# geobacter-rs/rav1e

Hardware: AMD Instinct MI355X
Metric: encoded frames/sec + Mpixels/sec, 4K 8-bit speed=10, 1/2/4/8 GPU vs host CPU (higher is better)
Workload: dtype u8

## Files before the change

### rav1e_amd/csrc/rv_chain.h

```cpp
#pragma once

#include "rv_device.h"

namespace rv {

__host__ __device__ inline rv_mv qfull(rv_mv m) {
  return rv_mv{(int16_t)((m.row / 8) * 8), (int16_t)((m.col / 8) * 8)};
}

__host__ __device__ inline rv_mc_job mc_job_for(const rv_plane &p, int po_x, int po_y, rv_mv mv,
                                       int dst_x, int dst_y) {
  const int ys = 3 + p.ydec, xs = 3 + p.xdec;
  const int roff = (int)mv.row >> ys, coff = (int)mv.col >> xs;
  rv_mc_job m;
  m.row_frac = ((int)mv.row - (roff << ys)) << (4 - ys);
  m.col_frac = ((int)mv.col - (coff << xs)) << (4 - xs);
  m.src_x = clampi(po_x + coff - 3, -p.xorigin, p.width) + 3;
  m.src_y = clampi(po_y + roff - 3, -p.yorigin, p.height) + 3;
  m.dst_x = dst_x;
  m.dst_y = dst_y;
  return m;
}

enum ChainMode {
// ... 4 lines not shown
struct ChainNext {
  int mode;
  rv_ds_job *jobs;
};

__device__ inline void chain_emit(const ChainNext &c, int job, int n_per_ref, int n_refs,
                                  rv_mv best) {
  (void)n_per_ref;
  (void)n_refs;
  if (c.mode == kChainFullToSub) c.jobs[job].pred[0] = best;
}

struct MvStack {
  int32_t n[2];
  rv_mv s[2][2];
  rv_mv c[2][2];
};

struct CandGeo {
  int nsb, tw, th, tx0, ty0, tws, ths;
  int R;
  int M;
  int comp;
  const MvStack *stk;
};

enum CandMode { kNearestMv = 0, kNear0Mv = 1, kGlobalMv = 2, kNewMv = 3, kCandModes = 4 };
enum CompMode {
  kGlobalGlobal = 0, kNearestNearest = 1, kNewNew = 2, kNearestNew = 3, kNewNearest = 4,
  kNearNear = 5, kCompModes = 6
};

__host__ __device__ inline bool mv_eq(rv_mv a, rv_mv b) { return a.row == b.row && a.col == b.col; }

__host__ __device__ inline int cand_stack(const CandGeo &g, const rv_fs_result *sub, int sb,
                                          int k, rv_mv &s0, rv_mv &s1) {
  if (g.stk) {
    const MvStack &m = g.stk[sb];
    s0 = m.s[k][0];
    s1 = m.s[k][1];
    return m.n[k];
  }
  const int sx = sb % g.tw, sy = sb / g.tw;
  const int fx = g.tx0 + sx, fy = g.ty0 + sy;
  const bool up = sy > 0 && fy % g.ths != 0, left = sx > 0 && fx % g.tws != 0;
  const rv_mv zero{0, 0};
  const rv_mv a = up ? sub[k * g.nsb + sb - g.tw].best_mv : zero;
  const rv_mv l = left ? sub[k * g.nsb + sb - 1].best_mv : zero;
  if (up) {
    s0 = a;
    s1 = l;
    return left && !mv_eq(l, a) ? 2 : 1;
  }
  s0 = l;
  s1 = zero;
  return left ? 1 : 0;
}

__host__ __device__ inline int comp_stack(const CandGeo &g, const rv_fs_result *sub, int sb,
                                          rv_mv &e00, rv_mv &e01, rv_mv &e10, rv_mv &e11) {
  if (g.stk) {
    const MvStack &m = g.stk[sb];
    e00 = m.c[0][0];
    e01 = m.c[0][1];
    e10 = m.c[1][0];
    e11 = m.c[1][1];
    return 2;
  }
  const int sx = sb % g.tw, sy = sb / g.tw;
  const int fx = g.tx0 + sx, fy = g.ty0 + sy;
  const bool up = sy > 0 && fy % g.ths != 0, left = sx > 0 && fx % g.tws != 0;
  const rv_mv zero{0, 0};
  const rv_mv a0 = up ? sub[sb - g.tw].best_mv : zero, a1 = up ? sub[g.nsb + sb - g.tw].best_mv : zero;
  const rv_mv l0 = left ? sub[sb - 1].best_mv : zero, l1 = left ? sub[g.nsb + sb - 1].best_mv : zero;
  e10 = e11 = zero;
  if (up) {
    e00 = a0;
    e01 = a1;
    if (left && (!mv_eq(l0, a0) || !mv_eq(l1, a1))) {
      e10 = l0;
      e11 = l1;
      return 2;
    }
    return 1;
  }
  e00 = l0;
  e01 = l1;
  return left ? 1 : 0;
}

__host__ __device__ inline void comp_mvs(const CandGeo &g, const rv_fs_result *sub, int sb, int m,
                                         rv_mv *mv0, rv_mv *mv1) {
  rv_mv e00, e01, e10, e11;
  const int n = comp_stack(g, sub, sb, e00, e01, e10, e11);
  const rv_mv zero{0, 0};
  const rv_mv me0 = sub[sb].best_mv, me1 = sub[g.nsb + sb].best_mv;
  const rv_mv n00 = n >= 1 ? e00 : zero, n01 = n >= 1 ? e01 : zero;
  switch (m) {
    case kGlobalGlobal:
      *mv0 = *mv1 = zero;
      break;
    case kNearestNearest:
      *mv0 = n00;
      *mv1 = n01;
      break;
    case kNewNew:
      *mv0 = me0;
      *mv1 = me1;
      break;
    case kNearestNew:
      *mv0 = n00;
      *mv1 = me1;
      break;
    case kNewNearest:
      *mv0 = me0;
      *mv1 = n01;
      break;
    default:
      *mv0 = n >= 2 ? e10 : zero;
      *mv1 = n >= 2 ? e11 : zero;
      break;
  }
}

__host__ __device__ inline bool cand_mv(const CandGeo &g, const rv_fs_result *sub, int sb, int c,
                                        rv_mv *mv) {
  const int k = c / g.M, m = c - k * g.M;
  rv_mv s0, s1;
  const int n = cand_stack(g, sub, sb, k, s0, s1);
  const rv_mv zero{0, 0};
  switch (m) {
    case kNearestMv:
      *mv = n >= 1 ? s0 : zero;
      return true;
    case kNear0Mv:
      *mv = n >= 2 ? s1 : zero;
      return n >= 1;
    case kGlobalMv:
      *mv = zero;
      return n >= 2;
    default: {
      const rv_mv me = sub[k * g.nsb + sb].best_mv;
      *mv = me;
      return !(n >= 1 && mv_eq(s0, me)) && !(n >= 2 && mv_eq(s1, me)) &&
             (me.row != 0 || me.col != 0);
    }
  }
}

__host__ __device__ inline bool cand_live(const CandGeo &g, const rv_fs_result *sub, int sb, int c,
                                          rv_mv *mv) {
  if (!cand_mv(g, sub, sb, c, mv)) return false;
  for (int c2 = (c / g.M) * g.M; c2 < c; c2++) {
    rv_mv m2;
    if (cand_mv(g, sub, sb, c2, &m2) && mv_eq(m2, *mv)) return false;
  }
  return true;
}
__host__ __device__ inline bool comp_live(const CandGeo &g, const rv_fs_result *sub, int sb, int m) {
  rv_mv a0, a1;
  comp_mvs(g, sub, sb, m, &a0, &a1);
  for (int m2 = 0; m2 < m; m2++) {
// ... 9 lines not shown
```

### rav1e_amd/csrc/rv_rdo.h

```cpp
#pragma once

#include "rv_chain.h"
#include "rv_device.h"
#include "rv_quant.h"

namespace rv {

struct RdoPlane {
  rv_plane org;
  rv_plane ref[2];
  rv_plane dst;
  int32_t *levels;
  uint64_t *out;
  QCtx q;
};

struct RdoWinner {
  int32_t c;
  int32_t skip;
  double cost;
  uint64_t dist;
};

struct RdoArgs {
// ... 6 lines not shown
  int n_tx;
  int cand_base;
  const int32_t *list;
  const int32_t *count;
  int commit;
  int ntx_per_cand;
  int bd;
  int bsize;
  int mb_w, mb_h;
  int sub_w, sub_h;
  int xdec, ydec;
  int q_tx_index;
  int tx_size, qindex;
  const void *iedges;
  const uint8_t *imodes;
  const uint8_t *iwin;
};

}

int rv_quant_ctx(int qindex, int tx_area, int is_intra, int bit_depth, int dc_delta_q,
                 int ac_delta_q, rv::QCtx *out);

int rv_rdo_candidates(const rv::RdoArgs &luma, const rv::RdoArgs &chroma, int hbd,
                      hipStream_t s, bool compound = false);

int rv_rdo_blocks2(const rv::RdoArgs &l, const rv::RdoArgs &c, int nl, int nc, int hbd,
                   hipStream_t s, int mode);
int rv_rdo_blocks(const rv::RdoArgs &a, bool luma, int nplanes, int n_tx_size, int hbd,
                  hipStream_t s, int mode);

int rv_rdo_args_put(const rv::RdoArgs *h, int n, rv::RdoArgs *dev, hipStream_t s);
int rv_rdo_candidates_list(const rv::RdoArgs *h, const rv::RdoArgs *dev, int nsets, int mode_a,
                           int hbd, hipStream_t s, int max_grid = 0, uint32_t *kp_cnt = nullptr,
                           unsigned long long *kp_t = nullptr);

int rv_rdo_intra(const rv::RdoArgs &luma, const rv::RdoArgs &chroma, int hbd, hipStream_t s);
```

### rav1e_amd/csrc/rv_rdo.hip

```cpp
#include <stdio.h>
#include <stdlib.h>
#include <string.h>

#include <type_traits>

#include "rv_distortion.h"
#include "rv_intra.h"
#include "rv_rdo.h"
#include "rv_tx.h"

namespace rv {


__constant__ int8_t kRdoReg[2][16][8] = {
    {{0, 0, 0, 127, 0, 0, 0, 0}, {0, 2, -6, 126, 8, -2, 0, 0},
     {0, 2, -10, 122, 18, -4, 0, 0}, {0, 2, -12, 116, 28, -8, 2, 0},
     {0, 2, -14, 110, 38, -10, 2, 0}, {0, 2, -14, 102, 48, -12, 2, 0},
     {0, 2, -16, 94, 58, -12, 2, 0}, {0, 2, -14, 84, 66, -12, 2, 0},
     {0, 2, -14, 76, 76, -14, 2, 0}, {0, 2, -12, 66, 84, -14, 2, 0},
     {0, 2, -12, 58, 94, -16, 2, 0}, {0, 2, -12, 48, 102, -14, 2, 0},
     {0, 2, -10, 38, 110, -14, 2, 0}, {0, 2, -8, 28, 116, -12, 2, 0},
     {0, 0, -4, 18, 122, -10, 2, 0}, {0, 0, -2, 8, 126, -6, 2, 0}},
    {{0, 0, 0, 127, 0, 0, 0, 0}, {0, 0, -4, 126, 8, -2, 0, 0},
     {0, 0, -8, 122, 18, -4, 0, 0}, {0, 0, -10, 116, 28, -6, 0, 0},
// ... 64 lines not shown
  const int tsx = fx % a.g.tws, tsy = fy % a.g.ths;
  j.ivar = tsx == 0 && tsy == 0 ? 0 : tsy == 0 ? 1 : tsx == 0 ? 2 : 3;
  j.imode = mode;
  j.iedge = (const uint8_t *)a.iedges + ((size_t)sb * 3 + plane) * kIntraEdge * sizeof(Px);
  j.bx = (fx * a.bsize) >> a.xdec;
  j.by = (fy * a.bsize) >> a.ydec;
  j.ox = j.oy = 0;
  j.src_x = j.src_y = j.cf = j.rf = j.ref = 0;
  j.src2_x = j.src2_y = j.cf2 = j.rf2 = 0;
  j.comp = false;
  j.zero = false;
  return j;
}

template <typename Px, int N, int G>
__device__ __forceinline__ void intra_fill(const RdoJob &jb, int32_t *e, Px *pred, int bd, int lane) {
  const Px *eg = (const Px *)jb.iedge;
  for (int i = lane; i < kIntraEdge; i += G) e[i] = eg[i];
  wave_sync();
  IntraSetup st = intra_setup(jb.imode, jb.ivar);
  if (st.mode == 0) st.dcv = intra_dc<G>(e, jb.ivar, N, N, bd, lane);
  const int maxv = (1 << bd) - 1;
  for (int i = lane; i < N * N; i += G) {
    const int r = i / N, c = i - r * N;
    pred[i] = (Px)intra_px(st, e, N, N, r, c, maxv);
  }
  wave_sync();
}

__device__ __forceinline__ int rdo_ntx(const RdoArgs &a) {
  return a.count ? __builtin_amdgcn_readfirstlane(*a.count) * a.ntx_per_cand : a.n_tx;
}

template <int N>
__device__ __forceinline__ RdoJob rdo_job(const RdoArgs &a, const RdoPlane &pl, int t) {
  const int ci = t / a.ntx_per_cand, sub = t - ci * a.ntx_per_cand;
  const int cand = a.list ? a.list[ci] : a.cand_base + ci;
  int sb, c;
  RdoJob j;
  j.zero = false;
  j.oi = cand * a.ntx_per_cand + sub;
  if (a.commit) {
    sb = cand;
    c = a.win[sb].c;
    j.zero = a.win[sb].skip != 0;
  } else {
    c = cand / a.g.nsb;
    sb = cand - c * a.g.nsb;
  }
  rv_mv mv, mv1{0, 0};
  j.comp = c >= a.g.R * a.g.M;
  if (j.comp) {
    comp_mvs(a.g, a.sub, sb, c - a.g.R * a.g.M, &mv, &mv1);
    j.ref = 0;
  } else {
    (void)cand_mv(a.g, a.sub, sb, c, &mv);
    j.ref = c / a.g.M;
  }
  const int sx = sb % a.g.tw, sy = sb / a.g.tw;
  j.bx = ((a.g.tx0 + sx) * a.bsize) >> a.xdec;
  j.by = ((a.g.ty0 + sy) * a.bsize) >> a.ydec;
  const int txc = a.mb_w / N;
  j.ox = (sub % txc) * N;
  j.oy = (sub / txc) * N;
  const rv_mc_job m = mc_job_for(pl.ref[j.ref], j.bx, j.by, mv, 0, 0);
  j.src_x = m.src_x;
  j.src_y = m.src_y;
  j.cf = m.col_frac;
  j.rf = m.row_frac;
  j.src2_x = j.src2_y = j.cf2 = j.rf2 = 0;
  if (j.comp) {
    const rv_mc_job m1 = mc_job_for(pl.ref[1], j.bx, j.by, mv1, 0, 0);
    j.src2_x = m1.src_x;
    j.src2_y = m1.src_y;
    j.cf2 = m1.col_frac;
    j.rf2 = m1.row_frac;
  }
  return j;
}

struct McF {
  uint32_t xp[3];
  int xsum;
  int yt[8];
  int cf, rf;
};
template <typename Px>
__device__ __forceinline__ McF mc_setup(int cf, int rf, int w, int h) {
  McF f;
// ... 181 lines not shown
        ss2 += (uint32_t)wmul24(sv, sv);
        sd2 += (uint32_t)wmul24(e, e);
        ssd += (uint32_t)wmul24(sv, e);
      }
#pragma unroll
      for (int m = 1; m < 8; m <<= 1) {
        ss += __shfl_xor(ss, m, 64);
        sd += __shfl_xor(sd, m, 64);
        ss2 += __shfl_xor(ss2, m, 64);
        sd2 += __shfl_xor(sd2, m, 64);
        ssd += __shfl_xor(ssd, m, 64);
      }
      if (row == 0) {
        const uint64_t v = cdef_dist_finish(ss, sd, ss2, sd2, ssd, a.bd);
        const int px = j.bx + j.ox + bx * 8, py = j.by + j.oy + by * 8;
        acc += distortion_biased(v, rdo_bias(a, px >> 2, py >> 2));
      }
    }
    return acc;
  } else {
    return rdo_sse_biased<Px, N, LPB>(a, j, o, os, d);
  }
}

template <typename Px, int N>
__host__ __device__ constexpr int rdo_slab_bytes() {
  constexpr int B = (int)sizeof(Px);
  constexpr int P = B == 1 ? ((N + 8 + 15) / 16) * 16 : ((2 * (N + 8) + 15) / 16) * 16;
  constexpr int RB = N < 16 ? N : 16;
  constexpr int a = N * (N + 1) * 4, b = (N + 7) * P, c = 2 * (RB + 7) * P;
  return ((a > b ? a : b) > c ? (a > b ? a : b) : c);
}

template <typename Px, int N, int LPB, int MODE, bool LUMA = false>
__device__ __forceinline__ void rdo_cand_body(const RdoArgs &a, const RdoPlane &pl, int t,
                                              bool valid, int32_t *buf, Px *pred,
                                              const uint16_t *scan) {
  constexpr int B = (int)sizeof(Px);
  constexpr int S = N + 1;
  constexpr int G = LPB / N, RG = N / G;
  constexpr int U = RG < 8 ? RG : 8;
  constexpr int P = B == 1 ? ((N + 8 + 15) / 16) * 16 : ((2 * (N + 8) + 15) / 16) * 16;
  constexpr int C32 = N < 32 ? N : 32;
  static_assert(!LUMA || N >= 8, "cdef distortion runs on 8x8 blocks");
  const int lane = rv_tid() & (LPB - 1);
  RdoJob jb;
  if constexpr (MODE == 3)
    jb = rdo_job_intra<Px, N>(a, &pl == &a.p[1] ? 2 : 1, t);
  else
    jb = rdo_job<N>(a, pl, t);
  const rv_plane &ref = pl.ref[jb.ref];
  const int ox = jb.ox, oy = jb.oy;
  const int bd = a.bd, ib = bd == 12 ? 2 : 4, maxv = (1 << bd) - 1;
  const int sx0 = jb.bx + ox, sy0 = jb.by + oy;
  auto wave_sync = [] {
    __builtin_amdgcn_fence(__ATOMIC_RELEASE, "wavefront");
    __builtin_amdgcn_wave_barrier();
    __builtin_amdgcn_fence(__ATOMIC_ACQUIRE, "wavefront");
  };

  if constexpr (MODE == 3) {
    intra_fill<Px, N, LPB>(jb, buf, pred, a.bd, lane);
  } else if (MODE == 1 || (MODE == 2 && jb.comp)) {
    static_assert(2 * (16 + 7) * (sizeof(Px) == 1 ? 48 : 80) <= N * (N + 1) * 4 || N != 32,
                  "compound windows must fit the coefficient slab");
    mc_compound<Px, N, (N < 16 ? N : 16)>(a, pl, jb, reinterpret_cast<uint32_t *>(buf), pred);
  } else
  {
    uint32_t *win = reinterpret_cast<uint32_t *>(buf);
    const uint8_t *sp = (const uint8_t *)plane_ptr<Px>(ref, jb.src_x + ox - 3, jb.src_y + oy - 3);
    const int64_t rs = (int64_t)ref.stride * B;
    constexpr int kRowDw = ((N + 7) * B + 3) / 4;
    constexpr int kTot = (N + 7) * kRowDw;
#pragma unroll 4
    for (int i = lane; i < kTot; i += LPB) {
      const int r = i / kRowDw, d = i - r * kRowDw;
      uint32_t v;
      __builtin_memcpy(&v, sp + r * rs + 4 * d, 4);
      win[r * (P / 4) + d] = B == 1 ? v ^ 0x80808080u : v;
    }
    wave_sync();
    const int cf = jb.cf, rf = jb.rf;
    const int8_t *xf = kRdoReg[a.mb_w <= 4][cf];
// ... 454 lines not shown
  }
  const uint64_t d = luma_dist<Px>(a, jb, plane_ptr<Px>(pl.org, jb.bx, jb.by), pl.org.stride, pred);
  if (valid && lane == 0) pl.out[(int64_t)jb.oi * 3 + 1] = d;
}

template <typename Px, typename Mid, int NPART, int MODE>
__device__ __forceinline__ void rdo_luma_body(const RdoArgs &a, const RdoPlane &pl, int t,
                                              uint8_t *scr, Px *pred, const uint16_t *scan) {
  const int lane = rv_tid() & 63;
  RdoJob jb;
  if constexpr (MODE == 3)
    jb = rdo_job_intra<Px, 64>(a, 0, t);
  else
    jb = rdo_job<64>(a, pl, t);
  luma_front<Px, NPART, MODE>(a, pl, t, jb, true, scr, pred);
  wave_sync();
  int32_t *fmid = reinterpret_cast<int32_t *>(scr);
  if (lane < 16) luma_fwd_row(fmid + lane * 65, a.bd);
  wave_sync();
  luma_quantize(a, pl, t, jb, true, fmid, scan);
  wave_sync();
  const int range = a.bd + 8, crange = a.bd + 6 > 16 ? a.bd + 6 : 16;
  Mid *imid = reinterpret_cast<Mid *>(scr);
  {
    int32_t v[64];
    if (lane < 32) luma_inv_row_load(fmid, lane, v, range, nullptr);
    wave_sync();
    if (lane < 32) luma_inv_row_tx(v, imid + lane * 66, range, crange);
  }
  wave_sync();
  luma_back<Px, Mid>(a, pl, t, jb, true, imid, pred);
}

template <typename Px, int MODE>
__device__ __forceinline__ void rdo_chroma_pair(const RdoArgs &chroma, int b, int32_t *buf,
                                                Px *pred, const uint16_t *scan, int pairs = -1) {
  if (pairs < 0) pairs = (chroma.n_tx + 1) / 2;
  const int plane = b / pairs;
  const int half = (rv_tid() & 63) >> 5;
  const int n = rdo_ntx(chroma);
  int i = 2 * (b - plane * pairs) + half;
  if (i - half >= n) return;
  const bool valid = i < n;
  if (!valid) i -= 1;
  rdo_cand_body<Px, 32, 32, MODE>(chroma, chroma.p[plane], i, valid, buf + half * 32 * 33,
                            pred + half * 32 * 32, scan);
}

__device__ __forceinline__ void stage_scan(uint16_t *dst, int tx_index) {
  const uint16_t *src = RV_SCANS + RV_SCAN_OFF[tx_index];
  for (int i = rv_tid(); i < 1024; i += blockDim.x) dst[i] = src[i];
  __syncthreads();
}

template <typename Px>
using SingleLds = LumaLds<Px, typename std::conditional<sizeof(Px) == 1, int16_t, int32_t>::type, 2>;
constexpr int kChromaPair(int pxb) { return 2 * 32 * 33 * 4 + 2 * 32 * 32 * pxb; }

template <typename Px, int MODE>
__global__ __launch_bounds__(64) __attribute__((amdgpu_waves_per_eu(4))) void rdo_frame_kernel(
    RdoArgs luma, RdoArgs chroma) {
  using L = SingleLds<Px>;
  using Mid = typename std::conditional<sizeof(Px) == 1, int16_t, int32_t>::type;
  __shared__ __align__(16) uint8_t lds[cmax(L::kSlot, kChromaPair(sizeof(Px)))];
  __shared__ uint16_t scan[1024];
  const int b = blockIdx.x;
  stage_scan(scan, b < luma.n_tx ? luma.q_tx_index : chroma.q_tx_index);
  if (b < luma.n_tx && b >= rdo_ntx(luma)) return;
  if (b < luma.n_tx)
    rdo_luma_body<Px, Mid, 2, MODE>(luma, luma.p[0], b, lds,
                              reinterpret_cast<Px *>(lds + L::kScr), scan);
  else
    rdo_chroma_pair<Px, MODE>(chroma, b - luma.n_tx, reinterpret_cast<int32_t *>(lds),
                        reinterpret_cast<Px *>(lds + 2 * 32 * 33 * 4), scan);
}

template <typename Px>
struct QuadLds {
  using L = LumaLds<Px, int16_t, sizeof(Px) == 1 ? 2 : 4>;
  static constexpr int kBytes = cmax(4 * L::kSlot, 3 * kChromaPair(sizeof(Px)));
};

#ifndef RV_RDO_PHASES
#define RV_RDO_PHASES 0
#endif
__device__ unsigned long long g_rdo_ph[3][8];
struct QuadPh {
  unsigned long long t[5];
};

template <typename Px, int MODE>
__device__ __forceinline__ void rdo_quad_luma(const RdoArgs &luma, int b, int n, int var,
                                              uint8_t *lds, const uint16_t *scan,
                                              QuadPh *ph = nullptr) {
  using L = typename QuadLds<Px>::L;
  constexpr int NPART = sizeof(Px) == 1 ? 2 : 4;
  const int wave = __builtin_amdgcn_readfirstlane(rv_tid() >> 6), lane = rv_tid() & 63;
  auto slot = [&](int q) __attribute__((always_inline)) { return lds + q * L::kSlot; };
  auto fmid = [&](int q) __attribute__((always_inline)) {
    return reinterpret_cast<int32_t *>(slot(q));
  };
  auto imid = [&](int q) __attribute__((always_inline)) {
    return reinterpret_cast<int16_t *>(slot(q));
  };
  auto pred = [&](int q) __attribute__((always_inline)) {
    return reinterpret_cast<Px *>(slot(q) + L::kScr);
  };
  const int t0 = 4 * b, t = t0 + wave;
  if (t0 >= n) return;
  const bool valid = t < n;
  RdoJob jb;
  if constexpr (MODE == 3)
    jb = rdo_job_intra<Px, 64>(luma, 0, valid ? t : n - 1);
  else
    jb = rdo_job<64>(luma, luma.p[0], valid ? t : n - 1);
  const bool late_dist = (var & 1) && !luma.commit;
  const bool prio = (var & 2) != 0;
  if (valid)
    luma_front<Px, NPART, MODE>(luma, luma.p[0], t, jb, true, slot(wave), pred(wave), !late_dist);
  __syncthreads();
  if (RV_RDO_PHASES && ph) ph->t[1] = wall_clock64();
  if (wave == 0) {
    if (prio) __builtin_amdgcn_s_setprio(2);
    const int q = lane >> 4;
    if (t0 + q < n) luma_fwd_row(fmid(q) + (lane & 15) * 65, luma.bd);
    if (prio) __builtin_amdgcn_s_setprio(0);
  } else if (late_dist && valid) {
    const uint64_t d = luma_dist<Px>(luma, jb, plane_ptr<Px>(luma.p[0].org, jb.bx, jb.by),
                                     luma.p[0].org.stride, pred(wave));
    if (lane == 0) luma.p[0].out[(int64_t)jb.oi * 3 + 0] = d;
  }
  __syncthreads();
  if (RV_RDO_PHASES && ph) ph->t[2] = wall_clock64();
  if (valid) luma_quantize(luma, luma.p[0], t, jb, true, fmid(wave), scan);
  __syncthreads();
  if (RV_RDO_PHASES && ph) ph->t[3] = wall_clock64();
  if (wave < 2) {
    if (prio) __builtin_amdgcn_s_setprio(2);
    const int q = 2 * wave + (lane >> 5), rr = lane & 31;
    const bool vq = t0 + q < n;
    const int range = luma.bd + 8, crange = luma.bd + 6 > 16 ? luma.bd + 6 : 16;
    int32_t v[64];
    if (vq) luma_inv_row_load(fmid(q), rr, v, range, nullptr);
    wave_sync();
    if (vq) luma_inv_row_tx(v, imid(q) + rr * 66, range, crange);
    if (prio) __builtin_amdgcn_s_setprio(0);
  } else if (wave == 2 && late_dist) {
    RdoJob j0;
    if constexpr (MODE == 3)
      j0 = rdo_job_intra<Px, 64>(luma, 0, t0);
    else
      j0 = rdo_job<64>(luma, luma.p[0], t0);
    const uint64_t d = luma_dist<Px>(luma, j0, plane_ptr<Px>(luma.p[0].org, j0.bx, j0.by),
                                     luma.p[0].org.stride, pred(0));
    if (lane == 0) luma.p[0].out[(int64_t)j0.oi * 3 + 0] = d;
  }
  __syncthreads();
  if (RV_RDO_PHASES && ph) ph->t[4] = wall_clock64();
  if (valid) luma_back<Px, int16_t>(luma, luma.p[0], t, jb, true, imid(wave), pred(wave));
}

template <typename Px, int MODE>
__device__ __forceinline__ void rdo_quad_chroma(const RdoArgs &chroma, int c, int pairs,
                                                uint8_t *lds, const uint16_t *scan) {
  const int wave = __builtin_amdgcn_readfirstlane(rv_tid() >> 6);
  const int pair = 3 * c + wave;
  if (wave == 3 || pair >= 2 * pairs) return;
  uint8_t *w = lds + wave * kChromaPair(sizeof(Px));
  rdo_chroma_pair<Px, MODE>(chroma, pair, reinterpret_cast<int32_t *>(w),
                            reinterpret_cast<Px *>(w + 2 * 32 * 33 * 4), scan, pairs);
}

template <typename Px, int MODE>
__device__ __forceinline__ void rdo_quad_chroma4(const RdoArgs &chroma, int c, int n, uint8_t *lds,
                                                 const uint16_t *scan) {
  constexpr int kSlab = rdo_slab_bytes<Px, 32>();
  static_assert(4 * (kSlab + 32 * 32 * (int)sizeof(Px)) <= QuadLds<Px>::kBytes, "4 chroma slabs");
  const int wave = __builtin_amdgcn_readfirstlane(rv_tid() >> 6);
  const int k = 4 * c + wave;
  if (k >= 2 * n) return;
  const int plane = k >= n ? 1 : 0, i = k - plane * n;
  uint8_t *w = lds + wave * (kSlab + 32 * 32 * (int)sizeof(Px));
  rdo_cand_body<Px, 32, 64, MODE>(chroma, chroma.p[plane], i, true, reinterpret_cast<int32_t *>(w),
                                  reinterpret_cast<Px *>(w + kSlab), scan);
}

template <typename Px, int MODE>
__device__ __forceinline__ void rdo_quad_wg(RdoArgs luma, RdoArgs chroma, int nquads,
                                            int var, int b, uint8_t *lds, uint16_t *scan) {
  if (b >= nquads) {
    const int pairs = (chroma.n_tx + 1) / 2, nc = rdo_ntx(chroma);
    bool any = false;
    for (int w = 0; w < 3; w++) {
      const int p = 3 * (b - nquads) + w;
      if (p < 2 * pairs) any |= 2 * (p - (p / pairs) * pairs) < nc;
    }
    if (!any) return;
  } else if (4 * b >= rdo_ntx(luma)) {
    return;
  }
  stage_scan(scan, b >= nquads ? chroma.q_tx_index : luma.q_tx_index);
  if (b >= nquads)
    rdo_quad_chroma<Px, MODE>(chroma, b - nquads, (chroma.n_tx + 1) / 2, lds, scan);
  else
    rdo_quad_luma<Px, MODE>(luma, b, rdo_ntx(luma), var, lds, scan);
}

template <typename Px, int MODE>
__global__ __launch_bounds__(256) __attribute__((amdgpu_waves_per_eu(4))) void rdo_quad_kernel(
    RdoArgs luma, RdoArgs chroma, int nquads, int var) {
  __shared__ __align__(16) uint8_t lds[QuadLds<Px>::kBytes];
  __shared__ uint16_t scan[1024];
  rdo_quad_wg<Px, MODE>(luma, chroma, nquads, var, blockIdx.x, lds, scan);
}

template <typename Px, int MA, int MB>
__global__ __launch_bounds__(256) __attribute__((amdgpu_waves_per_eu(4))) void rdo_quad_list_kernel(
    const RdoArgs *__restrict__ A, int nsets, int var, uint32_t *kp_cnt, unsigned long long *kp_t) {
  __shared__ __align__(16) uint8_t lds[QuadLds<Px>::kBytes];
  __shared__ uint16_t scan[1024];
  if (kp_t && threadIdx.x == 0) atomicMin(kp_t, (unsigned long long)wall_clock64());
  const RdoArgs &la = A[0], &ca = A[1], &lb = A[2], &cb = A[3];
  const int na = rdo_ntx(la), ma = rdo_ntx(ca);
  const int nb = nsets > 1 ? rdo_ntx(lb) : 0, mb = nsets > 1 ? rdo_ntx(cb) : 0;
  if (kp_cnt && blockIdx.x == 0 && threadIdx.x == 0) {
    atomicAdd(kp_cnt + (MA ? 1 : 0), (uint32_t)na);
    atomicAdd(kp_cnt + (MA ? 3 : 2), (uint32_t)ma);
    if (nsets > 1) {
      atomicAdd(kp_cnt + (MB ? 1 : 0), (uint32_t)nb);
      atomicAdd(kp_cnt + (MB ? 3 : 2), (uint32_t)mb);
    }
  }
  const int pa = (ma + 1) / 2, pb = (mb + 1) / 2;
  const bool c4 = (var & 32) != 0;
  const int e0 = (na + 3) / 4, e1 = e0 + (c4 ? (2 * ma + 3) / 4 : (2 * pa + 2) / 3);
  const int e2 = e1 + (nb + 3) / 4, e3 = e2 + (c4 ? (2 * mb + 3) / 4 : (2 * pb + 2) / 3);
  const bool phd = RV_RDO_PHASES && (var & 16) && rv_tid() == 0;
  for (int b = blockIdx.x; b < e3; b += gridDim.x) {
    QuadPh ph;
    ph.t[0] = phd ? wall_clock64() : 0;
    QuadPh *pp = phd ? &ph : nullptr;
    int set = 2;
    if (b < e0) {
      stage_scan(scan, la.q_tx_index);
      rdo_quad_luma<Px, MA>(la, b, na, var, lds, scan, pp);
      set = MA;
    } else if (b < e1) {
      stage_scan(scan, ca.q_tx_index);
      if (c4)
        rdo_quad_chroma4<Px, MA>(ca, b - e0, ma, lds, scan);
      else
        rdo_quad_chroma<Px, MA>(ca, b - e0, pa, lds, scan);
    } else if (b < e2) {
      stage_scan(scan, lb.q_tx_index);
      rdo_quad_luma<Px, MB>(lb, b - e1, nb, var, lds, scan, pp);
      set = MB;
    } else {
      stage_scan(scan, cb.q_tx_index);
      if (c4)
        rdo_quad_chroma4<Px, MB>(cb, b - e2, mb, lds, scan);
      else
        rdo_quad_chroma<Px, MB>(cb, b - e2, pb, lds, scan);
    }
    __syncthreads();
    if (phd) {
      const unsigned long long te = wall_clock64();
      if (set < 2) {
        for (int k = 0; k < 4; k++) atomicAdd(&g_rdo_ph[set][k], ph.t[k + 1] - ph.t[k]);
        atomicAdd(&g_rdo_ph[set][4], te - ph.t[4]);
      } else {
        atomicAdd(&g_rdo_ph[2][0], te - ph.t[0]);
      }
      atomicAdd(&g_rdo_ph[set][5], 1ull);
    }
  }
  if (kp_t && threadIdx.x == 0) atomicMax(kp_t + 1, (unsigned long long)wall_clock64());
}

__global__ __launch_bounds__(256) void rdo_args_store_kernel(RdoArgs a0, RdoArgs a1, RdoArgs a2,
                                                              RdoArgs a3, int n, RdoArgs *out) {
  static_assert(sizeof(RdoArgs) % 4 == 0, "word copy");
  constexpr int W = (int)(sizeof(RdoArgs) / 4);
  for (int i = threadIdx.x; i < n * W; i += blockDim.x) {
    const int k = i / W, w = i - k * W;
    const RdoArgs *s = k == 0 ? &a0 : k == 1 ? &a1 : k == 2 ? &a2 : &a3;
    uint32_t v;
    __builtin_memcpy(&v, reinterpret_cast<const uint8_t *>(s) + 4 * w, 4);
    __builtin_memcpy(reinterpret_cast<uint8_t *>(out + k) + 4 * w, &v, 4);
  }
}

constexpr unsigned kF4Pool = 1024;
constexpr int kRdoVariant = 3;

}

using namespace rv;

template <typename Px, int N, int MODE, bool LUMA>
__global__ __launch_bounds__(256) void rdo_small_kernel(RdoArgs a, int nplanes) {
  constexpr int TPW = 64 / N;
  constexpr int SLAB = rdo_slab_bytes<Px, N>();
  constexpr int PER = (SLAB + N * N * (int)sizeof(Px) + 15) / 16 * 16;
  __shared__ __align__(16) uint8_t lds[4 * TPW * PER];
  __shared__ uint16_t scan[1024];
  stage_scan(scan, a.q_tx_index);
  const int wave = rv_tid() >> 6, g = (rv_tid() & 63) / N;
  const int n = rdo_ntx(a), total = n * nplanes;
  const int w0 = (blockIdx.x * 4 + wave) * TPW;
  if (w0 >= total) return;
  const int i = w0 + g;
  const bool valid = i < total;
  const int ii = valid ? i : total - 1;
  const int plane = ii / n, t = ii - plane * n;
  uint8_t *mine = lds + (wave * TPW + g) * PER;
  rdo_cand_body<Px, N, N, MODE, LUMA>(a, a.p[plane], t, valid, reinterpret_cast<int32_t *>(mine),
                                       reinterpret_cast<Px *>(mine + SLAB), scan);
}

template <typename Px, int N, int MODE, bool LUMA>
__device__ __forceinline__ void rdo_small_part(const RdoArgs &a, int nplanes, int blk,
                                               uint8_t *lds, uint16_t *scan) {
  constexpr int TPW = 64 / N;
  constexpr int SLAB = rdo_slab_bytes<Px, N>();
  constexpr int PER = (SLAB + N * N * (int)sizeof(Px) + 15) / 16 * 16;
// ... 70 lines not shown
    return;
  }
  const int nquads = (luma.n_tx + 3) / 4;
  const unsigned grid = (unsigned)nquads + (cpairs + 2) / 3;
  if (grid == 0) return;
  if (hbd)
    rdo_quad_kernel<uint16_t, MODE><<<grid, 256, 0, s>>>(luma, chroma, nquads, kRdoVariant);
  else
    rdo_quad_kernel<uint8_t, MODE><<<grid, 256, 0, s>>>(luma, chroma, nquads, kRdoVariant);
}

int rv_rdo_candidates(const RdoArgs &luma, const RdoArgs &chroma, int hbd, hipStream_t s,
                      bool compound) {
  const unsigned cpairs = (unsigned)(2 * ((chroma.n_tx + 1) / 2));
  if (luma.commit)
    rdo_launch<2>(luma, chroma, hbd, s, cpairs);
  else if (compound)
    rdo_launch<1>(luma, chroma, hbd, s, cpairs);
  else
    rdo_launch<0>(luma, chroma, hbd, s, cpairs);
  RV_HIP_CHECK_LAUNCH();
  return RV_OK;
}

int rv_rdo_args_put(const RdoArgs *h, int n, RdoArgs *dev, hipStream_t s) {
  if (!h || !dev || n < 1 || n > 4) return rv_set_error(RV_EINVAL, "rv_rdo_args_put: bad arguments");
  rdo_args_store_kernel<<<1, 256, 0, s>>>(h[0], h[n > 1 ? 1 : 0], h[n > 2 ? 2 : 0], h[n > 3 ? 3 : 0],
                                          n, dev);
  RV_HIP_CHECK_LAUNCH();
  return RV_OK;
}

int rv_rdo_candidates_list(const RdoArgs *h, const RdoArgs *dev, int nsets, int mode_a, int hbd,
                           hipStream_t s, int max_grid, uint32_t *kp_cnt, unsigned long long *kp_t) {
  if (!h || !dev || nsets < 1 || nsets > 2 || mode_a < 0 || mode_a > 1 || (nsets == 2 && mode_a) ||
      h[0].commit || h[0].bd == 12)
    return rv_set_error(RV_EINVAL, "rv_rdo_candidates_list: bad arguments");
  for (int k = 0; k < 2 * nsets; k++)
    if (!h[k].list || !h[k].count)
      return rv_set_error(RV_EINVAL, "rv_rdo_candidates_list: the sets must be list-driven");
  static const bool phases = getenv("RAV1E_HIP_RDO_PHASES") && getenv("RAV1E_HIP_RDO_PHASES")[0] == '1';
  const int var = kRdoVariant | (phases && max_grid > 0 ? 16 : 0) | (max_grid > 0 ? 32 : 0);
  unsigned full = 0;
  for (int k = 0; k < nsets; k++)
    full += (unsigned)((h[2 * k].n_tx + 3) / 4) +
            ((var & 32) ? (unsigned)(2 * h[2 * k + 1].n_tx + 3) / 4
                        : (unsigned)(2 * ((h[2 * k + 1].n_tx + 1) / 2) + 2) / 3);
  unsigned grid = std::min(full, kF4Pool);
  if (max_grid > 0) grid = std::min(grid, (unsigned)max_grid);
  if (grid == 0) return RV_OK;
#define RV_LIST(PX, MA, MB) \
  rdo_quad_list_kernel<PX, MA, MB><<<grid, 256, 0, s>>>(dev, nsets, var, kp_cnt, kp_t)
  if (hbd) {
    if (nsets == 2) RV_LIST(uint16_t, 0, 1); else if (mode_a) RV_LIST(uint16_t, 1, 1); else RV_LIST(uint16_t, 0, 0);
  } else {
    if (nsets == 2) RV_LIST(uint8_t, 0, 1); else if (mode_a) RV_LIST(uint8_t, 1, 1); else RV_LIST(uint8_t, 0, 0);
  }
#undef RV_LIST
  RV_HIP_CHECK_LAUNCH();
  return RV_OK;
}

int rv_rdo_intra(const RdoArgs &luma, const RdoArgs &chroma, int hbd, hipStream_t s) {
  const unsigned cpairs = (unsigned)(2 * ((chroma.n_tx + 1) / 2));
  rdo_launch<3>(luma, chroma, hbd, s, cpairs);
  RV_HIP_CHECK_LAUNCH();
  return RV_OK;
}

int rv_rdo_blocks2(const RdoArgs &l, const RdoArgs &c, int nl, int nc, int hbd, hipStream_t s,
                   int mode) {
  if (nl == 32 && nc == 16) rdo_small2_launch<32, 16>(l, c, hbd, s, mode);
  else if (nl == 16 && nc == 8) rdo_small2_launch<16, 8>(l, c, hbd, s, mode);
  else if (nl == 8 && nc == 4) rdo_small2_launch<8, 4>(l, c, hbd, s, mode);
  else if (nl == 32 && nc == 32) rdo_small2_launch<32, 32>(l, c, hbd, s, mode);
  else if (nl == 16 && nc == 16) rdo_small2_launch<16, 16>(l, c, hbd, s, mode);
  else if (nl == 8 && nc == 8) rdo_small2_launch<8, 8>(l, c, hbd, s, mode);
  else return rv_set_error(RV_EINVAL, "rv_rdo_blocks2: sizes");
  RV_HIP_CHECK_LAUNCH();
  return RV_OK;
}

int rv_rdo_blocks(const RdoArgs &a, bool luma, int nplanes, int n_tx_size, int hbd,
                  hipStream_t s, int mode) {
  if (luma) {
    if (n_tx_size == 32) rdo_small_launch<32, true>(a, nplanes, hbd, s, mode);
    else if (n_tx_size == 16) rdo_small_launch<16, true>(a, nplanes, hbd, s, mode);
    else if (n_tx_size == 8) rdo_small_launch<8, true>(a, nplanes, hbd, s, mode);
    else return rv_set_error(RV_EINVAL, "rv_rdo_blocks: luma size");
// ... 32 lines not shown
```

### rav1e_amd/csrc/rv_replay_frame.hip

```cpp
#include "rv_replay.h"

namespace rv {

struct CandCost {
  double rs, rn;
  uint64_t ds, dn;
  int live;
};
__device__ inline CandCost cand_cost(const CandGeo &cg, double lambda, double ds_u, double ds_v,
                                     const rv_fs_result *sub, const uint64_t *lout,
                                     const uint64_t *uout, const uint64_t *vout, int ntx_c, int sb,
                                     int c) {
  CandCost k{0.0, 0.0, 0, 0, 0};
  const int ns = cg.R * cg.M;
  rv_mv mv;
  if (c < ns ? !cand_live(cg, sub, sb, c, &mv) : !comp_live(cg, sub, sb, c - ns)) return k;
  k.live = 1;
  const int64_t o = (int64_t)c * cg.nsb + sb;
  uint64_t su = 0, sv = 0, nu = 0, nv = 0;
  uint32_t rate = (uint32_t)lout[o * 3 + 2];
  for (int j = 0; j < ntx_c; j++) {
    const int64_t t = (o * ntx_c + j) * 3;
    su += uout[t];
    sv += vout[t];
// ... 972 lines not shown
      return rv_diamond_search_multi(&cur.hres, refs_h, g.R, r->jobs_half[lv], nr * 4, 16, 16, 0, 0,
                                     0, g.bd, r->half, nullptr, nullptr, st);
    RV_H(hipMemcpyAsync(r->half, r->half_l, (size_t)nr * g.R * 4 * sizeof(rv_fs_result),
                        hipMemcpyDeviceToDevice, st));
    fill_preds_kernel<<<(nr * g.R + 255) / 256, 256, 0, st>>>(r->jobs_full[lv], r->src_full,
                                                              nr * g.R, r->coarse, r->half, 0);
    return RV_OK;
  }

  int round0() {
    const bool with_lv = place == LvPlace::kRound0;
    if (f4_list) RV_R(rv_rdo_args_put(f4h, cg.comp ? 4 : 2, r->f4_args, st));
    RV_R(rv_diamond_search_multi(&cur.y, refs_y, g.R, r->jobs_full[lv], nr, 64, 64, 0, 0, 0, g.bd,
                                 r->full, ev_full, &to_sub, st, act));
    RV_R(ev(kEvF3Full));
    RV_R(kp.open(st));
    RV_R(rv_diamond_search_multi(&cur.y, refs_y, g.R, r->jobs_sub[lv], nr, 64, 64, 1,
                                 r->s6 ? 1 : 0, 0, g.bd, r->sub, ev_sub, nullptr, st, act, nullptr,
                                 nullptr, 1, nullptr, 0, kp.acc(0), kp.ts()));
    RV_R(kp.close(st));
    if (with_lv) RV_R(lv_me(st));
    const CandKeys keys0{r->cand_key, (uint32_t)(r->coded + 1), 0};
    cand_list_kernel<<<(nsingle + 255) / 256, 256, 0, st>>>(cg, r->sub, nsingle, r->cand_list,
                                                            r->cand_count, act, keys0);
    if (with_lv) lv_lists(st, false);
    if (cg.comp) {
      comp_list_kernel<<<(g.nsb * cg.comp + 255) / 256, 256, 0, st>>>(
          cg, r->sub, nsingle, r->cand_list + nsingle, r->cand_count + 1, act, keys0);
      if (with_lv) lv_lists(st, true);
    }
    RV_R(ev(kEvF3Sub));
    if (f4_list) {
      RV_R(kp.open(st, 1));
      RV_R(rv_rdo_candidates_list(f4h, r->f4_args, 1, 0, g.hbd, st, 0, kp.acc(1), kp.ts(1)));
      RV_R(kp.close(st, 1));
    } else
      RV_R(rv_rdo_candidates(f4h[0], f4h[1], g.hbd, st));
    if (with_lv) RV_R(lv_rdo(st));
    RV_R(ev(kEvF4Single));
    if (cg.comp) {
      if (f4_list) {
        RV_R(kp.open(st, 1));
        RV_R(rv_rdo_candidates_list(f4h + 2, r->f4_args + 2, 1, 1, g.hbd, st, 0, kp.acc(1), kp.ts(1)));
        RV_R(kp.close(st, 1));
      } else
        RV_R(rv_rdo_candidates(f4h[2], f4h[3], g.hbd, st, true));
      if (with_lv) RV_R(lv_rdo_comp(st));
    }
    RV_R(ev(kEvF4Comp));
    score_wave_kernel<<<(g.nsb + 3) / 4, 256, 0, st>>>(
        g, cg, L.lambda, L.ds[1], L.ds[2], r->sub, r->l_out, r->c_out, r->c_out + nct * 3, ntx_c,
        r->win, r->coarse, r->half, r->full, r->look, r->half_l, r->words, r->cand_count,
        r->tail + 2, r->cand_evals + 2 * slot * kLevels, r->leaf_count, nullptr, nullptr,
        r->exact ? r->dec_lv[lv] : nullptr, 0);
    return RV_OK;
  }

  int round_of(uint32_t q) {
    const int32_t *acnt = slot_cnt(q);
    int lg = q == q_first ? nr * g.R : 0;
    const int hint = q == q_first ? -1 : r->rr.last_count;
    const int hsb = hint >= 0 ? std::max(2 * hint, 16) : 0;
    int f4_grid = 0;
    if (hsb) {
      lg = std::min(hsb * g.R, 512);
      f4_grid = std::min(6 * hsb, 1024);
    }
    RV_R(kp.open(st));
    RV_R(rv_diamond_f2_f3(&cur.hres, refs_h, r->jobs_half[lv], r->half, ma.f2dirty, &cur.y,
                          refs_y, r->jobs_full[lv], r->full, ma.f3dirty, &to_sub, g.R, nr, g.bd,
                          mvl(q), acnt, lg, st, r->jobs_sub[lv], r->sub, kp.acc(0), kp.ts()));
    RV_R(kp.close(st));
    const int rg = hsb ? std::min(kRoundGrid, std::max((14 * hsb + 255) / 256, (hsb + 3) / 4))
                       : kRoundGrid;
    round_lists_kernel<<<rg, 256, 0, st>>>(
        cg, r->sub, nsingle, r->cand_list, r->cand_count, mvl(q), acnt,
        CandKeys{r->cand_key, (uint32_t)(r->coded + 1), 1});
    if (f4_list) {
      RV_R(kp.open(st, 1));
      RV_R(rv_rdo_candidates_list(f4h, r->f4_args, cg.comp ? 2 : 1, 0, g.hbd, st, f4_grid,
                                  kp.acc(1), kp.ts(1)));
      RV_R(kp.close(st, 1));
    } else {
      RV_R(rv_rdo_candidates(f4h[0], f4h[1], g.hbd, st));
      if (cg.comp) RV_R(rv_rdo_candidates(f4h[2], f4h[3], g.hbd, st, true));
    }
    score_wave_kernel<<<rg, 256, 0, st>>>(
        g, cg, L.lambda, L.ds[1], L.ds[2], r->sub, r->l_out, r->c_out, r->c_out + nct * 3, ntx_c,
        r->win, r->coarse, r->half, r->full, r->look, r->half_l, r->words, r->cand_count, nullptr,
        nullptr, nullptr, mvl(q), acnt, r->dec_lv[lv], 1);
    return RV_OK;
  }

  int mv_rounds_run(const uint8_t *iwas, bool *changed) {
    mv_runs++;
    q_first = r->rr.seq;
    ma.init = 0;
    ma.iwas = iwas;
    return run_rounds(
        r->rr, st, budget, [this](uint32_t q) { return check(q); },
        [this](uint32_t q) { return round_of(q); }, &r->mv_round_sum, &r->mv_reeval, changed,
        "mvref", ncoded, lv);
  }
  int rounds() {
    RV_R(join_edge_scores());
    ma.hq = r->half;
    ma.edge_ok = 1;
    tr.r0 = HostTrace::now();
    RV_R(mv_rounds_run(nullptr, nullptr));
    tr.mv = HostTrace::now();
    return RV_OK;
  }

  PartArgs part_args() const {
// ... 258 lines not shown
```

Baseline: 179.0.

## Add latency-mode F4 list kernel with lower wave occupancy and branchless MV stacks

Adds a latency variant of the RDO candidate list kernel, used for 8-bit non-first motion rounds. It compiles with amdgpu_waves_per_eu(2) instead of 4 and caps the grid at 768 workgroups instead of 1024. That variant also builds the neighbour MV stacks branchlessly through a templated BV path, which computes both candidates and selects between them rather than branching. The aim is to give each wave more registers and cut divergence and latency in the small later rounds, at the cost of fewer concurrent waves.

```diff
diff --git a/rav1e_amd/csrc/rv_chain.h b/rav1e_amd/csrc/rv_chain.h
--- a/rav1e_amd/csrc/rv_chain.h
+++ b/rav1e_amd/csrc/rv_chain.h
@@ -60,7 +60,13 @@
 };
 
 __host__ __device__ inline bool mv_eq(rv_mv a, rv_mv b) { return a.row == b.row && a.col == b.col; }
-
+__host__ __device__ inline rv_mv mv_if(bool c, const rv_mv &m) {
+  rv_mv r{0, 0};
+  if (c) r = m;
+  return r;
+}
+
+template <bool BV = false>
 __host__ __device__ inline int cand_stack(const CandGeo &g, const rv_fs_result *sub, int sb,
                                           int k, rv_mv &s0, rv_mv &s1) {
   if (g.stk) {
@@ -73,6 +79,13 @@
   const int fx = g.tx0 + sx, fy = g.ty0 + sy;
   const bool up = sy > 0 && fy % g.ths != 0, left = sx > 0 && fx % g.tws != 0;
   const rv_mv zero{0, 0};
+  if constexpr (BV) {
+    const rv_mv a = mv_if(up, sub[k * g.nsb + sb - g.tw].best_mv);
+    const rv_mv l = mv_if(left, sub[k * g.nsb + sb - 1].best_mv);
+    s0 = up ? a : l;
+    s1 = up ? l : zero;
+    return up ? (left && !mv_eq(l, a) ? 2 : 1) : left ? 1 : 0;
+  }
   const rv_mv a = up ? sub[k * g.nsb + sb - g.tw].best_mv : zero;
   const rv_mv l = left ? sub[k * g.nsb + sb - 1].best_mv : zero;
   if (up) {
@@ -85,6 +98,7 @@
   return left ? 1 : 0;
 }
 
+template <bool BV = false>
 __host__ __device__ inline int comp_stack(const CandGeo &g, const rv_fs_result *sub, int sb,
                                           rv_mv &e00, rv_mv &e01, rv_mv &e10, rv_mv &e11) {
   if (g.stk) {
@@ -99,8 +113,14 @@
   const int fx = g.tx0 + sx, fy = g.ty0 + sy;
   const bool up = sy > 0 && fy % g.ths != 0, left = sx > 0 && fx % g.tws != 0;
   const rv_mv zero{0, 0};
-  const rv_mv a0 = up ? sub[sb - g.tw].best_mv : zero, a1 = up ? sub[g.nsb + sb - g.tw].best_mv : zero;
-  const rv_mv l0 = left ? sub[sb - 1].best_mv : zero, l1 = left ? sub[g.nsb + sb - 1].best_mv : zero;
+  rv_mv a0, a1, l0, l1;
+  if constexpr (BV) {
+    a0 = mv_if(up, sub[sb - g.tw].best_mv), a1 = mv_if(up, sub[g.nsb + sb - g.tw].best_mv);
+    l0 = mv_if(left, sub[sb - 1].best_mv), l1 = mv_if(left, sub[g.nsb + sb - 1].best_mv);
+  } else {
+    a0 = up ? sub[sb - g.tw].best_mv : zero, a1 = up ? sub[g.nsb + sb - g.tw].best_mv : zero;
+    l0 = left ? sub[sb - 1].best_mv : zero, l1 = left ? sub[g.nsb + sb - 1].best_mv : zero;
+  }
   e10 = e11 = zero;
   if (up) {
     e00 = a0;
@@ -117,10 +137,11 @@
   return left ? 1 : 0;
 }
 
+template <bool BV = false>
 __host__ __device__ inline void comp_mvs(const CandGeo &g, const rv_fs_result *sub, int sb, int m,
                                          rv_mv *mv0, rv_mv *mv1) {
   rv_mv e00, e01, e10, e11;
-  const int n = comp_stack(g, sub, sb, e00, e01, e10, e11);
+  const int n = comp_stack<BV>(g, sub, sb, e00, e01, e10, e11);
   const rv_mv zero{0, 0};
   const rv_mv me0 = sub[sb].best_mv, me1 = sub[g.nsb + sb].best_mv;
   const rv_mv n00 = n >= 1 ? e00 : zero, n01 = n >= 1 ? e01 : zero;
@@ -151,11 +172,12 @@
   }
 }
 
+template <bool BV = false>
 __host__ __device__ inline bool cand_mv(const CandGeo &g, const rv_fs_result *sub, int sb, int c,
                                         rv_mv *mv) {
   const int k = c / g.M, m = c - k * g.M;
   rv_mv s0, s1;
-  const int n = cand_stack(g, sub, sb, k, s0, s1);
+  const int n = cand_stack<BV>(g, sub, sb, k, s0, s1);
   const rv_mv zero{0, 0};
   switch (m) {
     case kNearestMv:
diff --git a/rav1e_amd/csrc/rv_rdo.h b/rav1e_amd/csrc/rv_rdo.h
--- a/rav1e_amd/csrc/rv_rdo.h
+++ b/rav1e_amd/csrc/rv_rdo.h
@@ -62,7 +62,7 @@
 
 int rv_rdo_args_put(const rv::RdoArgs *h, int n, rv::RdoArgs *dev, hipStream_t s);
 int rv_rdo_candidates_list(const rv::RdoArgs *h, const rv::RdoArgs *dev, int nsets, int mode_a,
-                           int hbd, hipStream_t s, int max_grid = 0, uint32_t *kp_cnt = nullptr,
-                           unsigned long long *kp_t = nullptr);
+                           int hbd, hipStream_t s, int max_grid = 0, bool latency = false,
+                           uint32_t *kp_cnt = nullptr, unsigned long long *kp_t = nullptr);
 
 int rv_rdo_intra(const rv::RdoArgs &luma, const rv::RdoArgs &chroma, int hbd, hipStream_t s);
diff --git a/rav1e_amd/csrc/rv_rdo.hip b/rav1e_amd/csrc/rv_rdo.hip
--- a/rav1e_amd/csrc/rv_rdo.hip
+++ b/rav1e_amd/csrc/rv_rdo.hip
@@ -120,7 +120,7 @@
   return a.count ? __builtin_amdgcn_readfirstlane(*a.count) * a.ntx_per_cand : a.n_tx;
 }
 
-template <int N>
+template <int N, bool BV = false>
 __device__ __forceinline__ RdoJob rdo_job(const RdoArgs &a, const RdoPlane &pl, int t) {
   const int ci = t / a.ntx_per_cand, sub = t - ci * a.ntx_per_cand;
   const int cand = a.list ? a.list[ci] : a.cand_base + ci;
@@ -139,10 +139,10 @@
   rv_mv mv, mv1{0, 0};
   j.comp = c >= a.g.R * a.g.M;
   if (j.comp) {
-    comp_mvs(a.g, a.sub, sb, c - a.g.R * a.g.M, &mv, &mv1);
+    comp_mvs<BV>(a.g, a.sub, sb, c - a.g.R * a.g.M, &mv, &mv1);
     j.ref = 0;
   } else {
-    (void)cand_mv(a.g, a.sub, sb, c, &mv);
+    (void)cand_mv<BV>(a.g, a.sub, sb, c, &mv);
     j.ref = c / a.g.M;
   }
   const int sx = sb % a.g.tw, sy = sb / a.g.tw;
@@ -390,7 +390,7 @@
   return ((a > b ? a : b) > c ? (a > b ? a : b) : c);
 }
 
-template <typename Px, int N, int LPB, int MODE, bool LUMA = false>
+template <typename Px, int N, int LPB, int MODE, bool LUMA = false, bool BV = false>
 __device__ __forceinline__ void rdo_cand_body(const RdoArgs &a, const RdoPlane &pl, int t,
                                               bool valid, int32_t *buf, Px *pred,
                                               const uint16_t *scan) {
@@ -406,7 +406,7 @@
   if constexpr (MODE == 3)
     jb = rdo_job_intra<Px, N>(a, &pl == &a.p[1] ? 2 : 1, t);
   else
-    jb = rdo_job<N>(a, pl, t);
+    jb = rdo_job<N, BV>(a, pl, t);
   const rv_plane &ref = pl.ref[jb.ref];
   const int ox = jb.ox, oy = jb.oy;
   const int bd = a.bd, ib = bd == 12 ? 2 : 4, maxv = (1 << bd) - 1;
@@ -927,7 +927,7 @@
   luma_back<Px, Mid>(a, pl, t, jb, true, imid, pred);
 }
 
-template <typename Px, int MODE>
+template <typename Px, int MODE, bool BV = false>
 __device__ __forceinline__ void rdo_chroma_pair(const RdoArgs &chroma, int b, int32_t *buf,
                                                 Px *pred, const uint16_t *scan, int pairs = -1) {
   if (pairs < 0) pairs = (chroma.n_tx + 1) / 2;
@@ -938,7 +938,7 @@
   if (i - half >= n) return;
   const bool valid = i < n;
   if (!valid) i -= 1;
-  rdo_cand_body<Px, 32, 32, MODE>(chroma, chroma.p[plane], i, valid, buf + half * 32 * 33,
+  rdo_cand_body<Px, 32, 32, MODE, false, BV>(chroma, chroma.p[plane], i, valid, buf + half * 32 * 33,
                             pred + half * 32 * 32, scan);
 }
 
@@ -984,7 +984,7 @@
   unsigned long long t[5];
 };
 
-template <typename Px, int MODE>
+template <typename Px, int MODE, bool BV = false>
 __device__ __forceinline__ void rdo_quad_luma(const RdoArgs &luma, int b, int n, int var,
                                               uint8_t *lds, const uint16_t *scan,
                                               QuadPh *ph = nullptr) {
@@ -1008,7 +1008,7 @@
   if constexpr (MODE == 3)
     jb = rdo_job_intra<Px, 64>(luma, 0, valid ? t : n - 1);
   else
-    jb = rdo_job<64>(luma, luma.p[0], valid ? t : n - 1);
+    jb = rdo_job<64, BV>(luma, luma.p[0], valid ? t : n - 1);
   const bool late_dist = (var & 1) && !luma.commit;
   const bool prio = (var & 2) != 0;
   if (valid)
@@ -1045,7 +1045,7 @@
     if constexpr (MODE == 3)
       j0 = rdo_job_intra<Px, 64>(luma, 0, t0);
     else
-      j0 = rdo_job<64>(luma, luma.p[0], t0);
+      j0 = rdo_job<64, BV>(luma, luma.p[0], t0);
     const uint64_t d = luma_dist<Px>(luma, j0, plane_ptr<Px>(luma.p[0].org, j0.bx, j0.by),
                                      luma.p[0].org.stride, pred(0));
     if (lane == 0) luma.p[0].out[(int64_t)j0.oi * 3 + 0] = d;
@@ -1055,18 +1055,18 @@
   if (valid) luma_back<Px, int16_t>(luma, luma.p[0], t, jb, true, imid(wave), pred(wave));
 }
 
-template <typename Px, int MODE>
+template <typename Px, int MODE, bool BV = false>
 __device__ __forceinline__ void rdo_quad_chroma(const RdoArgs &chroma, int c, int pairs,
                                                 uint8_t *lds, const uint16_t *scan) {
   const int wave = __builtin_amdgcn_readfirstlane(rv_tid() >> 6);
   const int pair = 3 * c + wave;
   if (wave == 3 || pair >= 2 * pairs) return;
   uint8_t *w = lds + wave * kChromaPair(sizeof(Px));
-  rdo_chroma_pair<Px, MODE>(chroma, pair, reinterpret_cast<int32_t *>(w),
+  rdo_chroma_pair<Px, MODE, BV>(chroma, pair, reinterpret_cast<int32_t *>(w),
                             reinterpret_cast<Px *>(w + 2 * 32 * 33 * 4), scan, pairs);
 }
 
-template <typename Px, int MODE>
+template <typename Px, int MODE, bool BV = false>
 __device__ __forceinline__ void rdo_quad_chroma4(const RdoArgs &chroma, int c, int n, uint8_t *lds,
                                                  const uint16_t *scan) {
   constexpr int kSlab = rdo_slab_bytes<Px, 32>();
@@ -1076,7 +1076,7 @@
   if (k >= 2 * n) return;
   const int plane = k >= n ? 1 : 0, i = k - plane * n;
   uint8_t *w = lds + wave * (kSlab + 32 * 32 * (int)sizeof(Px));
-  rdo_cand_body<Px, 32, 64, MODE>(chroma, chroma.p[plane], i, true, reinterpret_cast<int32_t *>(w),
+  rdo_cand_body<Px, 32, 64, MODE, false, BV>(chroma, chroma.p[plane], i, true, reinterpret_cast<int32_t *>(w),
                                   reinterpret_cast<Px *>(w + kSlab), scan);
 }
 
@@ -1109,9 +1109,10 @@
   rdo_quad_wg<Px, MODE>(luma, chroma, nquads, var, blockIdx.x, lds, scan);
 }
 
-template <typename Px, int MA, int MB>
-__global__ __launch_bounds__(256) __attribute__((amdgpu_waves_per_eu(4))) void rdo_quad_list_kernel(
+template <typename Px, int MA, int MB, int WAVES>
+__global__ __launch_bounds__(256) __attribute__((amdgpu_waves_per_eu(WAVES))) void rdo_quad_list_kernel(
     const RdoArgs *__restrict__ A, int nsets, int var, uint32_t *kp_cnt, unsigned long long *kp_t) {
+  constexpr bool BV = WAVES != 4;
   __shared__ __align__(16) uint8_t lds[QuadLds<Px>::kBytes];
   __shared__ uint16_t scan[1024];
   if (kp_t && threadIdx.x == 0) atomicMin(kp_t, (unsigned long long)wall_clock64());
@@ -1138,24 +1139,24 @@
     int set = 2;
     if (b < e0) {
       stage_scan(scan, la.q_tx_index);
-      rdo_quad_luma<Px, MA>(la, b, na, var, lds, scan, pp);
+      rdo_quad_luma<Px, MA, BV>(la, b, na, var, lds, scan, pp);
       set = MA;
     } else if (b < e1) {
       stage_scan(scan, ca.q_tx_index);
       if (c4)
-        rdo_quad_chroma4<Px, MA>(ca, b - e0, ma, lds, scan);
+        rdo_quad_chroma4<Px, MA, BV>(ca, b - e0, ma, lds, scan);
       else
-        rdo_quad_chroma<Px, MA>(ca, b - e0, pa, lds, scan);
+        rdo_quad_chroma<Px, MA, BV>(ca, b - e0, pa, lds, scan);
     } else if (b < e2) {
       stage_scan(scan, lb.q_tx_index);
-      rdo_quad_luma<Px, MB>(lb, b - e1, nb, var, lds, scan, pp);
+      rdo_quad_luma<Px, MB, BV>(lb, b - e1, nb, var, lds, scan, pp);
       set = MB;
     } else {
       stage_scan(scan, cb.q_tx_index);
       if (c4)
-        rdo_quad_chroma4<Px, MB>(cb, b - e2, mb, lds, scan);
+        rdo_quad_chroma4<Px, MB, BV>(cb, b - e2, mb, lds, scan);
       else
-        rdo_quad_chroma<Px, MB>(cb, b - e2, pb, lds, scan);
+        rdo_quad_chroma<Px, MB, BV>(cb, b - e2, pb, lds, scan);
     }
     __syncthreads();
     if (phd) {
@@ -1185,7 +1186,7 @@
   }
 }
 
-constexpr unsigned kF4Pool = 1024;
+constexpr unsigned kF4Pool = 1024, kF4PoolLat = 768;
 constexpr int kRdoVariant = 3;
 
 }
@@ -1322,7 +1323,8 @@
 }
 
 int rv_rdo_candidates_list(const RdoArgs *h, const RdoArgs *dev, int nsets, int mode_a, int hbd,
-                           hipStream_t s, int max_grid, uint32_t *kp_cnt, unsigned long long *kp_t) {
+                           hipStream_t s, int max_grid, bool latency, uint32_t *kp_cnt,
+                           unsigned long long *kp_t) {
   if (!h || !dev || nsets < 1 || nsets > 2 || mode_a < 0 || mode_a > 1 || (nsets == 2 && mode_a) ||
       h[0].commit || h[0].bd == 12)
     return rv_set_error(RV_EINVAL, "rv_rdo_candidates_list: bad arguments");
@@ -1336,15 +1338,17 @@
     full += (unsigned)((h[2 * k].n_tx + 3) / 4) +
             ((var & 32) ? (unsigned)(2 * h[2 * k + 1].n_tx + 3) / 4
                         : (unsigned)(2 * ((h[2 * k + 1].n_tx + 1) / 2) + 2) / 3);
-  unsigned grid = std::min(full, kF4Pool);
+  unsigned grid = std::min(full, latency && !hbd ? kF4PoolLat : kF4Pool);
   if (max_grid > 0) grid = std::min(grid, (unsigned)max_grid);
   if (grid == 0) return RV_OK;
-#define RV_LIST(PX, MA, MB) \
-  rdo_quad_list_kernel<PX, MA, MB><<<grid, 256, 0, s>>>(dev, nsets, var, kp_cnt, kp_t)
+#define RV_LIST(PX, MA, MB, W) \
+  rdo_quad_list_kernel<PX, MA, MB, W><<<grid, 256, 0, s>>>(dev, nsets, var, kp_cnt, kp_t)
   if (hbd) {
-    if (nsets == 2) RV_LIST(uint16_t, 0, 1); else if (mode_a) RV_LIST(uint16_t, 1, 1); else RV_LIST(uint16_t, 0, 0);
+    if (nsets == 2) RV_LIST(uint16_t, 0, 1, 4); else if (mode_a) RV_LIST(uint16_t, 1, 1, 4); else RV_LIST(uint16_t, 0, 0, 4);
+  } else if (latency && !mode_a) {
+    if (nsets == 2) RV_LIST(uint8_t, 0, 1, 2); else RV_LIST(uint8_t, 0, 0, 2);
   } else {
-    if (nsets == 2) RV_LIST(uint8_t, 0, 1); else if (mode_a) RV_LIST(uint8_t, 1, 1); else RV_LIST(uint8_t, 0, 0);
+    if (nsets == 2) RV_LIST(uint8_t, 0, 1, 4); else if (mode_a) RV_LIST(uint8_t, 1, 1, 4); else RV_LIST(uint8_t, 0, 0, 4);
   }
 #undef RV_LIST
   RV_HIP_CHECK_LAUNCH();
diff --git a/rav1e_amd/csrc/rv_replay_frame.hip b/rav1e_amd/csrc/rv_replay_frame.hip
--- a/rav1e_amd/csrc/rv_replay_frame.hip
+++ b/rav1e_amd/csrc/rv_replay_frame.hip
@@ -1028,7 +1028,7 @@
     RV_R(ev(kEvF3Sub));
     if (f4_list) {
       RV_R(kp.open(st, 1));
-      RV_R(rv_rdo_candidates_list(f4h, r->f4_args, 1, 0, g.hbd, st, 0, kp.acc(1), kp.ts(1)));
+      RV_R(rv_rdo_candidates_list(f4h, r->f4_args, 1, 0, g.hbd, st, 0, false, kp.acc(1), kp.ts(1)));
       RV_R(kp.close(st, 1));
     } else
       RV_R(rv_rdo_candidates(f4h[0], f4h[1], g.hbd, st));
@@ -1037,7 +1037,8 @@
     if (cg.comp) {
       if (f4_list) {
         RV_R(kp.open(st, 1));
-        RV_R(rv_rdo_candidates_list(f4h + 2, r->f4_args + 2, 1, 1, g.hbd, st, 0, kp.acc(1), kp.ts(1)));
+        RV_R(rv_rdo_candidates_list(f4h + 2, r->f4_args + 2, 1, 1, g.hbd, st, 0, false, kp.acc(1),
+                                    kp.ts(1)));
         RV_R(kp.close(st, 1));
       } else
         RV_R(rv_rdo_candidates(f4h[2], f4h[3], g.hbd, st, true));
@@ -1075,7 +1076,7 @@
     if (f4_list) {
       RV_R(kp.open(st, 1));
       RV_R(rv_rdo_candidates_list(f4h, r->f4_args, cg.comp ? 2 : 1, 0, g.hbd, st, f4_grid,
-                                  kp.acc(1), kp.ts(1)));
+                                  q != q_first, kp.acc(1), kp.ts(1)));
       RV_R(kp.close(st, 1));
     } else {
       RV_R(rv_rdo_candidates(f4h[0], f4h[1], g.hbd, st));
```

Result: no change. 178.8 (-0.1%).
